# zchuning/repo

Measured on AMD Instinct MI355X. Metric: world-model+imagine updates/sec (B=50,L=50,64x64x3), higher is better.
Workload: dtype f32

## Files before the change

### include/repo_hip.h

```cpp
#ifndef REPO_HIP_H
#define REPO_HIP_H

#include <stddef.h>
#include <stdint.h>

#ifdef __cplusplus
extern "C" {
#endif

#ifndef __HIP_PLATFORM_AMD__
typedef struct ihipStream_t* hipStream_t;
#endif

#define REPO_ABI_VERSION 14

#define REPO_OK 0
#define REPO_E_BADARG (-1)
#define REPO_E_SHAPE (-2)
#define REPO_E_ALIGN (-3)
#define REPO_E_WS_TOO_SMALL (-4)
#define REPO_E_ARCH (-5)
#define REPO_E_ENV (-6)

#define REPO_EPI_NONE 0
// ... 277 lines not shown
int repo_vdb_head_bwd(int64_t N, int64_t Z, const float* z, int64_t ldz, const float* eps, uint64_t noise_seed,
                      uint64_t noise_offset, const float* lat, const float* fc_w, const float* dd, const float* beta,
                      float kl_coef, const float* extra, float* dz, int64_t lddz, float* dfc_w, float* dfc_b,
                      int accumulate, void* ws, size_t ws_bytes, hipStream_t stream);
int repo_vdb_beta_step(float* beta, const float* kl_real_sum, int64_t n_real, const float* kl_fake_sum, int64_t n_fake,
                       float beta_lr, float target_kl, float* kl_out, hipStream_t stream);
int repo_vdb_gp_delta(int64_t N, int64_t Z, const float* z, int64_t ldz, const float* eps, uint64_t noise_seed,
                      uint64_t noise_offset, const float* lat, const float* fc_w, float* delta5, int64_t lddelta,
                      hipStream_t stream);
int repo_vdb_gp_norm(int64_t n, float* g, float scale, float* sq_sum, void* ws, size_t ws_bytes, hipStream_t stream);
int repo_vdb_gp_head(int64_t N, int64_t Z, const float* a5, int64_t lda5, const float* z, int64_t ldz, const float* eps,
                     uint64_t noise_seed, uint64_t noise_offset, const float* lat, const float* fc_w, float* extra,
                     float* dfc_w, int accumulate, void* ws, size_t ws_bytes, hipStream_t stream);
int repo_vdb_tau(int64_t N, const float* lt, const float* d, const float* u, float* tau_out, float* dlt, float* sums,
                 void* ws, size_t ws_bytes, hipStream_t stream);

int repo_linear_unit_nll_fused(int64_t rows, int64_t O, int64_t K, const float* h, int64_t ldh, const float* W,
                               int64_t ldw);
int repo_linear_unit_nll(int64_t rows, int64_t O, int64_t K, const float* h, int64_t ldh, const float* W, int64_t ldw,
                         const float* bias, const float* target, int64_t ldt, float grad_scale, float* sums, float* dpre,
                         int64_t lddpre, float* recon, int64_t ldrecon, float* scratch, size_t scratch_bytes, void* ws,
                         size_t ws_bytes, hipStream_t stream);
int repo_debug_linear_nll(int mode);

int repo_film_fwd(int64_t nimg, int64_t C, int64_t P, const float* y, const float* film, int64_t ldfilm,
                  int64_t gamma_off, int64_t beta_off, float* out, hipStream_t stream);
int repo_film_bwd(int64_t nimg, int64_t C, int64_t P, const float* dh, const float* y, const float* film,
                  int64_t ldfilm, int64_t gamma_off, int64_t beta_off, float* dy, float* dfilm, hipStream_t stream);
int repo_film_tables(int64_t nimg, int nlayers, const int* channels, const float* film, int64_t ldfilm, float* tables,
                     hipStream_t stream);
int repo_film_bwd_h(int64_t nimg, int64_t C, int64_t P, const float* dh, const float* h, const float* film,
                    int64_t ldfilm, int64_t gamma_off, int64_t beta_off, float* dy, float* dfilm, int conv_kind,
                    const int64_t* geo, const void* x, int x_is_u8, const float* w, const float* bias,
                    unsigned* gated_epoch, unsigned epoch, hipStream_t stream);
size_t repo_kl_balance_tasks_workspace_bytes(void);
int repo_kl_balance_tasks(int64_t rows, int64_t S, int64_t C, const float* pm, const float* ps, const float* qm,
                          const float* qs, float alpha, const float* log_beta, const float* tasks, float target_kl,
                          float scale, float* dpm, float* dps, float* dqm, float* dqs, float* sums, void* ws,
                          size_t ws_bytes, hipStream_t stream);
int repo_dual_step_tasks(int64_t C, float* log_beta, float* exp_avg, float* exp_avg_sq, const float* sums,
                         int64_t rows, float lr, float beta1, float beta2, float eps, int64_t step, int apply,
                         float* scalars_out, const unsigned* skip_if_nonzero, hipStream_t stream);

int repo_transpose(int64_t rows, int64_t cols, const float* src, int64_t lds, float* dst, int64_t ldd,
                   hipStream_t stream);
int repo_gemm_nt_pays(int64_t M, int64_t N, int64_t K);

size_t repo_grad_sqnorm_workspace_bytes(void);
int repo_grad_sqnorm(int64_t n, const float* g, float* sqnorm, void* ws, size_t ws_bytes,
                     hipStream_t stream);
int repo_clip_adam(int64_t n, float* params, const float* grads, float* exp_avg, float* exp_avg_sq,
                   const float* sqnorm, float max_norm, float lr, float beta1, float beta2, float eps,
                   int64_t step, const unsigned* skip_if_nonzero, hipStream_t stream);

#ifdef __cplusplus
}
#endif
#endif
```

### repo_amd/algorithms/repo/dreamer.py

```python
import functools
import glob
import math
import os

import numpy as np
import torch

from ... import functional as Fn
from ... import ops
from ...common.buffers import SequenceReplayBuffer
from ...common.utils import get_device, postprocess, to_np
from .models.actor_critic import ActorModel, ValueModel
from .models.decoder import ContinuationModel, ObservationModel, RewardModel
from .models.encoder import Encoder
from .models.rssm import TransitionModel
from .models.utils import FlatAdam, InverseDynamicsModel
from .rollout import EpisodeDriver

LOG_2PI = math.log(2.0 * math.pi)


def _d(ts):
    return [t.detach() for t in ts]

# ... 279 lines not shown
        if self._pcont:
            self._pcont_backward(feat, st["pc_hid"], st["dpc"], dfeat)
        pd, gd = self._pg(self.obs_model)
        pr, gr = self._pg(self.transition_model)
        pe, ge = self._pg(self.encoder)
        dembeds = torch.empty(rows, self.c.embedding_size, device=dev)
        dpm, dps, dqm, dqs = kl_grads
        if self._symbolic:
            Fn.symbolic_decoder_bwd(pd, feat, st["dec_saved"], gd, self.obs_model.act,
                                    dfeat=dfeat if decoder_attached else None, accumulate_dfeat=True)
            self._model_bucket_begin(tail=True)
            ops.rssm_observe_bwd(pr, sv, gr, dfeat=dfeat, dpm=dpm, dps=dps, dqm=dqm, dqs=dqs, dembeds=dembeds,
                                 min_std=self.transition_model.min_std_dev)
            Fn.symbolic_encoder_bwd(pe, st["frames"], st["enc_saved"], dembeds, ge, self.encoder.act)
            return
        if decoder_attached:
            wgrads = []
            Fn.decoder_bwd(pd, feat, st["dec_saved"], gd, dfeat=dfeat, accumulate_dfeat=True, deferred=wgrads)
            main = torch.cuda.current_stream(dev)
            side = self._side_stream or main
            side.wait_stream(main)
            with torch.cuda.stream(side):
                ops.rssm_observe_bwd(pr, sv, gr, dfeat=dfeat, dpm=dpm, dps=dps, dqm=dqm, dqs=dqs, dembeds=dembeds,
                                     min_std=self.transition_model.min_std_dev)
            for fn in wgrads:
                fn()
            main.wait_stream(side)
            self._model_bucket_begin(tail=True)
            Fn.encoder_bwd(pe, st["frames"], st["enc_saved"], dembeds, ge, side=wside)
            return
        main = torch.cuda.current_stream(dev)
        side = self._side_stream or main
        side.wait_stream(main)
        with torch.cuda.stream(side):
            ops.rssm_observe_bwd(pr, sv, gr, dfeat=dfeat, dpm=dpm, dps=dps, dqm=dqm, dqs=dqs, dembeds=dembeds,
                                 min_std=self.transition_model.min_std_dev)
        Fn.decoder_bwd(pd, feat, st["dec_saved"], gd, side=wside)
        main.wait_stream(side)
        self._model_bucket_begin(tail=True)
        Fn.encoder_bwd(pe, st["frames"], st["enc_saved"], dembeds, ge, side=wside)

    def _model_bucket_begin(self, tail):
        if self.dp is None or not self._dp_two_buckets:
            return
        g, cut = self.model_optimizer.grad, self._model_cut
        if not tail:
            self._allreduce(g[:cut])
            return
        self._model_works.append(self.dp.all_reduce_begin(g[cut:], stream=self._side_stream))

    def _steppers(self):
        return [v for v in vars(self).values() if hasattr(v, "step_count") and hasattr(v, "exp_avg")]

    def _take_status(self):
        st = self._status_ring[self._update_seq % 8 : self._update_seq % 8 + 1]
        ops.take_status_into(ops.scan_status(self.device), st)
        if self.dp is not None:
            self.dp.all_reduce_status(st)
        self._ustatus = st
        for opt in self._steppers():
            opt.skip = st
        return st

    def _model_step(self):
        self._take_status()
        if self._ev_ac_done is not None:
            torch.cuda.current_stream(self.device).wait_event(self._ev_ac_done)
        if self.dp is not None and self._dp_two_buckets:
            self._model_bucket_begin(tail=False)
            works, self._model_works = self._model_works, []
            assert len(works) == 1, "model gradient buckets: the decoder bucket was not started by the backward"
            self.dp.all_reduce_end(works)
        elif self.dp is not None:
            self._allreduce(self.model_optimizer.grad)
        self.model_optimizer.clip_and_step(self.c.grad_clip_norm)

    def _prep_batch(self, obs, actions, rewards, nonterms):
        self._update_seq += 1
        self._restore_point = (self._update_seq, self._noise_counter, [(o, o.step_count) for o in self._steppers()])
        obs = obs.contiguous()
        assert obs.dtype in (torch.uint8, torch.float32), obs.dtype
        return obs, actions.float().contiguous(), rewards.float().contiguous(), nonterms.float().contiguous()

    @in_conv_precision
    def train_dynamics(self, obs, actions, rewards, nonterms):
        c = self.c
        obs, actions, rewards, nonterms = self._prep_batch(obs, actions, rewards, nonterms)
        st = self._world_model_forward(obs, actions, rewards, nonterms)
        sv, grow = st["sv"], st["grow"]
        if sv.prior_ready is not None:
            torch.cuda.current_stream(self.device).wait_stream(sv.prior_ready)
        kl_sum, kl_grads = ops.kl_balance(sv.prior_mean, sv.prior_std, sv.post_mean, sv.post_std, 1, 0.0, None,
                                          float(c.free_nats), 1.0 / grow)
        self._world_model_backward(st, kl_grads, decoder_attached=True)
        self._model_step()
        self._pending_model = (torch.cat([st["nll_sum"], st["rew_sums"], kl_sum, self.model_optimizer.sqnorm]), None,
                               grow)
        return self._latents_out(sv, actions, nonterms)

    def _latents_out(self, sv, actions, nonterms):
        D = self.c.belief_size
        beliefs, states = sv.featx[1:, :, :D], sv.featx[1:, :, D:]
        if self._inv_dyn:
            self.train_inv_dynamics(beliefs, states, actions, nonterms)
        return beliefs, states

    def train_inv_dynamics(self, beliefs, states, actions, nonterms):
        c = self.c
        m, opt = self.inv_dynamics, self.inv_dynamics_optimizer
        T, B, D = beliefs.shape
        S = states.shape[2]
        rows = beliefs.as_strided((T, B, D + S), beliefs.stride()) if (
            states.data_ptr() == beliefs.data_ptr() + 4 * D and states.stride() == beliefs.stride()
            and beliefs.stride(1) >= D + S) else torch.cat((beliefs, states), dim=2)
        x = ops.inv_dyn_pack(rows, D)
        N = x.shape[0]
        p, g = self._pg(m)
        raw, hid = ops.mlp_fwd(p, x, act=m.act)
        target, mask = actions[1:-1].reshape(N, -1), nonterms[1:-1].reshape(N)
        if self.dp is None:
            sums, draw = ops.normal_nll_rows(raw, target, mask, m.min_std_dev)
        else:
            sums, _ = ops.normal_nll_rows(raw, target, mask, m.min_std_dev, want_grad=False)
            total = sums.clone()
            self._allreduce(total)
            _, draw = ops.normal_nll_rows(raw, target, mask, m.min_std_dev, count_in=total[1:2])
        ops.mlp_bwd(p, x, hid, draw, dparams=g, dx=None, act=m.act)
        self._allreduce(opt.grad)
# ... 432 lines not shown
```

### repo_amd/algorithms/repo/models/utils.py

```python
import torch
import torch.nn as nn
import torch.nn.functional as F

from .... import ops


def bottle(f, xs):
    horizon, batch_size = xs[0].shape[:2]
    ys = f(*(x.reshape(horizon * batch_size, *x.shape[2:]) for x in xs))
    if isinstance(ys, tuple):
        return tuple(y.reshape(horizon, batch_size, *y.shape[1:]) for y in ys)
    return ys.reshape(horizon, batch_size, *ys.shape[1:])


class InverseDynamicsModel(nn.Module):

    def __init__(self, belief_size, state_size, action_size, hidden_size, activation_function="relu", min_std_dev=0.1):
        super().__init__()
        self.act = ops.dense_act_id(activation_function, type(self).__name__)
        self.min_std_dev = min_std_dev
        self.fc1 = nn.Linear(belief_size + state_size + belief_size, hidden_size)
        self.fc2 = nn.Linear(hidden_size, hidden_size)
        self.fc3 = nn.Linear(hidden_size, hidden_size)
        self.fc4 = nn.Linear(hidden_size, 2 * action_size)

    def plist(self):
        return [t for m in (self.fc1, self.fc2, self.fc3, self.fc4) for t in (m.weight, m.bias)]

    @torch.no_grad()
    def forward(self, belief, state, next_belief):
        x = torch.cat((belief, state, next_belief), dim=1).float().contiguous()
        raw, _ = ops.mlp_fwd([t.detach() for t in self.plist()], x, act=self.act)
        mean, std_dev = torch.chunk(raw, chunks=2, dim=1)
        return mean, F.softplus(std_dev) + self.min_std_dev


def adam_param_group(lr, betas, eps, n_params):
    probe = torch.optim.Adam([torch.nn.Parameter(torch.zeros(1))], lr=float(lr), betas=tuple(betas), eps=float(eps))
    group = dict(probe.state_dict()["param_groups"][0])
    group["params"] = list(range(n_params))
    return group


class FlatAdam:

    @staticmethod
    def padded_numel(params):
        return sum((p.numel() + 3) // 4 * 4 for p in params)

    def __init__(self, params, lr, betas=(0.9, 0.999), eps=1e-8, grad=None):
        self.params = list(params)
        assert self.params, "FlatAdam needs at least one parameter"
        self.lr, self.betas, self.eps = float(lr), tuple(betas), float(eps)
        self.step_count = 0
        dev = self.params[0].device
        sizes = [p.numel() for p in self.params]
        self.offsets, off = [], 0
        for n in sizes:
            self.offsets.append(off)
            off += (n + 3) // 4 * 4
        self.numel = off
        self.flat = torch.zeros(off, dtype=torch.float32, device=dev)
        if grad is None:
            grad = torch.zeros(off, dtype=torch.float32, device=dev)
        assert grad.shape == (off,) and grad.dtype == torch.float32 and grad.is_contiguous(), (grad.shape, off)
        self.grad = grad
        self.exp_avg = torch.zeros(off, dtype=torch.float32, device=dev)
        self.exp_avg_sq = torch.zeros(off, dtype=torch.float32, device=dev)
        self.sqnorm = torch.zeros(1, dtype=torch.float32, device=dev)
        self.skip = None
        self.gviews = []
        with torch.no_grad():
            for p, o, n in zip(self.params, self.offsets, sizes):
                self.flat[o : o + n].copy_(p.detach().reshape(-1))
                p.data = self.flat[o : o + n].view(p.shape)
                gv = self.grad[o : o + n].view(p.shape)
                p.grad = gv
                self.gviews.append(gv)

    @classmethod
    def view(cls, parent, n_params, lr):
        self = cls.__new__(cls)
        self.params = parent.params[:n_params]
        self.lr, self.betas, self.eps = float(lr), parent.betas, parent.eps
        self.step_count = 0
        self.offsets = parent.offsets[:n_params]
        self.numel = parent.offsets[n_params] if n_params < len(parent.params) else parent.numel
        self.flat, self.grad = parent.flat[: self.numel], parent.grad[: self.numel]
        self.exp_avg = torch.zeros_like(self.flat)
        self.exp_avg_sq = torch.zeros_like(self.flat)
        self.sqnorm = torch.zeros(1, dtype=torch.float32, device=self.flat.device)
        self.skip = None
        self.gviews = parent.gviews[:n_params]
        return self

    def zero_grad(self, set_to_none=False):
        self.grad.zero_()

    def clip_and_step(self, max_norm):
        self.step_count += 1
        ops.grad_sqnorm(self.grad, out=self.sqnorm)
        ops.clip_adam(self.flat, self.grad, self.exp_avg, self.exp_avg_sq, self.sqnorm, max_norm, self.lr,
                      self.step_count, self.betas, self.eps, skip=self.skip)

    def step(self):
        self.step_count += 1
        ops.clip_adam(self.flat, self.grad, self.exp_avg, self.exp_avg_sq, None, 0.0, self.lr, self.step_count,
                      self.betas, self.eps, skip=self.skip)

    def state_dict(self):
        state = {}
        if self.step_count > 0:
            for i, (p, o) in enumerate(zip(self.params, self.offsets)):
                n = p.numel()
                state[i] = {
                    "step": torch.tensor(float(self.step_count)),
                    "exp_avg": self.exp_avg[o : o + n].view(p.shape).clone(),
                    "exp_avg_sq": self.exp_avg_sq[o : o + n].view(p.shape).clone(),
                }
        return {"state": state, "param_groups": [adam_param_group(self.lr, self.betas, self.eps, len(self.params))]}

    def load_state_dict(self, sd):
        g = sd["param_groups"][0]
        self.lr, self.betas, self.eps = float(g["lr"]), tuple(g["betas"]), float(g["eps"])
        steps = set()
        with torch.no_grad():
            for i, (p, o) in enumerate(zip(self.params, self.offsets)):
                st = sd["state"].get(i)
                if st is None:
                    continue
                n = p.numel()
                self.exp_avg[o : o + n].copy_(st["exp_avg"].reshape(-1))
                self.exp_avg_sq[o : o + n].copy_(st["exp_avg_sq"].reshape(-1))
                steps.add(int(float(st["step"])))
        assert len(steps) <= 1, "per-parameter step counts differ; not an Adam state this optimiser can hold"
        self.step_count = steps.pop() if steps else 0
```

### repo_amd/algorithms/repo/repo.py

```python
import os

import numpy as np
import torch

from ... import functional as Fn
from ... import ops
from .dreamer import Dreamer, in_conv_precision
from .models.utils import adam_param_group


class _ScalarAdam:

    def __init__(self, param, lr, betas=(0.9, 0.999), eps=1e-8):
        self.param = param
        self.lr, self.betas, self.eps = float(lr), tuple(betas), float(eps)
        self.step_count = 0
        self.exp_avg = torch.zeros(1, dtype=torch.float32, device=param.device)
        self.exp_avg_sq = torch.zeros(1, dtype=torch.float32, device=param.device)

    def state_dict(self):
        state = {}
        if self.step_count > 0:
            state[0] = {"step": torch.tensor(float(self.step_count)), "exp_avg": self.exp_avg.reshape(()).clone(),
                        "exp_avg_sq": self.exp_avg_sq.reshape(()).clone()}
# ... 14 lines not shown
        super().build_models(config, env)
        self.log_beta = torch.tensor(np.log(config.init_beta), dtype=torch.float, device=self.device)
        self.beta_optimizer = _ScalarAdam(self.log_beta, lr=self.c.beta_lr)
        self._dual_out = torch.zeros(4, dtype=torch.float32, device=self.device)

    def _train_dynamics_split(self, obs, actions, rewards, nonterms):
        c, dev = self.c, self.device
        L, B = obs.shape[:2]
        T = L - 1
        rows = T * B
        grow = self._global_rows(rows)
        D, S = c.belief_size, c.state_size
        frames = obs[1:].reshape(rows, *obs.shape[2:])
        pe, ge = self._pg(self.encoder)
        embeds, enc_saved = Fn.encoder_fwd(pe, frames)
        pr, gr = self._pg(self.transition_model)
        pd, gd = self._pg(self.obs_model)
        head = Fn.dec_head_compose(pd) if Fn._dec_compose(rows, pd) else None
        sv = ops.rssm_observe_fwd(
            pr, *self._zero_state(B), actions[:-1].contiguous(),
            nonterms[:-1].reshape(T, B).contiguous(), embeds.view(T, B, -1), self._noise("obs_prior", (T, B, S)),
            self._noise("obs_post", (T, B, S)), self.transition_model.min_std_dev, noise=self._draw(2 * T * B * S),
            act=self.transition_model.act)
        feat = sv.featx[1:].reshape(rows, D + S)
        pw, gw = self._pg(self.reward_model)
        r_pred, r_hid = ops.mlp_fwd(pw, feat, act=self.reward_model.act)
        rew_sums, drew = ops.scalar_nll(r_pred.view(-1), rewards[:-1].reshape(-1).contiguous(),
                                        nonterms[:-1].reshape(-1).contiguous(), 1.0 / grow)
        if self._pcont:
            pc_hid, dpc = self._pcont_forward(feat, nonterms, grow)
        alpha = c.prior_train_steps / (1 + c.prior_train_steps)
        kl_sum, klg = ops.kl_balance(sv.prior_mean, sv.prior_std, sv.post_mean, sv.post_std, 0, alpha, self.log_beta, 0.0,
                                     1.0 / grow)
        main, side = torch.cuda.current_stream(dev), self._side_stream
        side.wait_stream(main)
        with torch.cuda.stream(side):
            dfeat = torch.empty(rows, D + S, device=dev)
            ops.mlp_bwd(pw, feat, r_hid, drew.view(rows, 1), dparams=gw, dx=dfeat, act=self.reward_model.act)
            if self._pcont:
                self._pcont_backward(feat, pc_hid, dpc, dfeat)
            ev_rew = torch.cuda.Event()
            ev_rew.record(side)
            dembeds = torch.empty(rows, c.embedding_size, device=dev)
            ops.rssm_observe_bwd(pr, sv, gr, dfeat=dfeat, dpm=klg[0], dps=klg[1], dqm=klg[2], dqs=klg[3], dembeds=dembeds,
                                 min_std=self.transition_model.min_std_dev)
            Fn.encoder_bwd(pe, frames, enc_saved, dembeds, ge, side=None)
        nll_sum, dec_saved = Fn.decoder_fwd_nll(pd, feat, frames, 1.0 / grow, head=head)
        Fn.decoder_bwd(pd, feat, dec_saved, gd, side=self._wgrad_side(B))
        if self.dp is not None and self._dp_two_buckets:
            main.wait_event(ev_rew)
            g, cut = self.model_optimizer.grad, self._model_cut
            self._model_works.append(self.dp.all_reduce_begin(g[cut:], stream=main))
        main.wait_stream(side)
        self._model_step()
        kl_global = kl_sum
        if self.dp is not None:
            kl_global = kl_sum.clone()
            self._allreduce(kl_global)
        bo = self.beta_optimizer
        bo.step_count += 1
        ops.dual_step(self.log_beta, bo.exp_avg, bo.exp_avg_sq, kl_global, grow, c.target_kl, bo.lr, bo.step_count,
                      betas=bo.betas, eps=bo.eps, out=self._dual_out, skip=self._ustatus)
        self._pending_model = (torch.cat([nll_sum, rew_sums, kl_sum, self.model_optimizer.sqnorm]), self._dual_out.clone(),
                               grow)
        return self._latents_out(sv, actions, nonterms)

    @in_conv_precision
    def train_dynamics(self, obs, actions, rewards, nonterms):
        c = self.c
        obs, actions, rewards, nonterms = self._prep_batch(obs, actions, rewards, nonterms)
        if os.environ.get("REPO_WM_SPLIT", "1") == "1" and self._side_stream is not None and not self._symbolic:
            return self._train_dynamics_split(obs, actions, rewards, nonterms)
        st = self._world_model_forward(obs, actions, rewards, nonterms)
        sv, grow = st["sv"], st["grow"]
        alpha = c.prior_train_steps / (1 + c.prior_train_steps)
        if sv.prior_ready is not None:
            torch.cuda.current_stream(self.device).wait_stream(sv.prior_ready)
        kl_sum, kl_grads = ops.kl_balance(sv.prior_mean, sv.prior_std, sv.post_mean, sv.post_std, 0, alpha,
                                          self.log_beta, 0.0, 1.0 / grow)
        self._world_model_backward(st, kl_grads, decoder_attached=False)
        self._model_step()
        kl_global = kl_sum
        if self.dp is not None:
            kl_global = kl_sum.clone()
            self._allreduce(kl_global)
        bo = self.beta_optimizer
        bo.step_count += 1
        ops.dual_step(self.log_beta, bo.exp_avg, bo.exp_avg_sq, kl_global, grow, c.target_kl, bo.lr, bo.step_count,
                      betas=bo.betas, eps=bo.eps, out=self._dual_out, skip=self._ustatus)
        self._pending_model = (torch.cat([st["nll_sum"], st["rew_sums"], kl_sum, self.model_optimizer.sqnorm]),
                               self._dual_out.clone(), grow)
        return self._latents_out(sv, actions, nonterms)

    def get_param_dict(self):
        params = super().get_param_dict()
        params["log_beta"] = self.log_beta.detach().clone().requires_grad_(True)
        params["beta_optimizer"] = self.beta_optimizer.state_dict()
        return params

    def load_param_dict(self, params):
        super().load_param_dict(params)
        with torch.no_grad():
            self.log_beta.copy_(params["log_beta"].to(self.device))
        self.beta_optimizer.load_state_dict(params["beta_optimizer"])
```

### repo_amd/csrc/common.h

```cpp
#pragma once
#include <hip/hip_runtime.h>
#include <stdint.h>

#include "../../include/repo_hip.h"

#define REPO_CHECK_LAUNCH()                      \
  do {                                           \
    hipError_t _e = hipGetLastError();           \
    if (_e != hipSuccess) return (int)_e;        \
  } while (0)

#define REPO_ARCH_GUARD()                 \
  do {                                    \
    int _a = repo::arch_status();         \
    if (_a != REPO_OK) return _a;         \
  } while (0)

#define REPO_REQUIRE(cond, code) \
  do {                           \
    if (!(cond)) return (code);  \
  } while (0)

namespace repo {

// ... 26 lines not shown
__device__ __forceinline__ float pix_norm(uint8_t v) { return ((float)v / 255.f) * 2.f - 1.f; }

__device__ __forceinline__ float load_as_float(const float* p, unsigned i) { return p[i]; }
__device__ __forceinline__ float load_as_float(const uint8_t* p, unsigned i) { return pix_norm(p[i]); }

__device__ __forceinline__ float wave_sum(float v) {
#pragma unroll
  for (int o = 32; o > 0; o >>= 1) v += __shfl_xor(v, o, 64);
  return v;
}
__device__ __forceinline__ double wave_sum_d(double v) {
#pragma unroll
  for (int o = 32; o > 0; o >>= 1) v += __shfl_xor(v, o, 64);
  return v;
}

__device__ __forceinline__ float block_sum(float v, float* smem ) {
  v = wave_sum(v);
  const int lane = threadIdx.x & 63, wid = threadIdx.x >> 6;
  if (lane == 0) smem[wid] = v;
  __syncthreads();
  float r = 0.f;
  if (threadIdx.x == 0) {
    const int nw = (blockDim.x + 63) >> 6;
    for (int i = 0; i < nw; ++i) r += smem[i];
  }
  __syncthreads();
  return r;
}

constexpr int kRedHeaderBytes = 256;
constexpr int kLastBlockMaxGrid = 64;
__device__ __forceinline__ void last_block_finishes(const float* parts, int nvals, float* out, unsigned* ticket, float* smem) {
  if (!ticket) return;
  __shared__ int s_last;
  __threadfence();
  __syncthreads();
  if (threadIdx.x == 0)
    s_last = __hip_atomic_fetch_add(ticket, 1u, __ATOMIC_RELAXED, __HIP_MEMORY_SCOPE_AGENT) == gridDim.x - 1;
  __syncthreads();
  if (!s_last) return;
  __threadfence();
  const int n = gridDim.x;
  for (int v = 0; v < nvals; ++v) {
    float s = 0.f;
    for (int i = threadIdx.x; i < n; i += blockDim.x)
      s += __hip_atomic_load(parts + v * n + i, __ATOMIC_RELAXED, __HIP_MEMORY_SCOPE_AGENT);
    s = block_sum(s, smem);
    if (threadIdx.x == 0) out[v] = s;
  }
  if (threadIdx.x == 0) __hip_atomic_store(ticket, 0u, __ATOMIC_RELAXED, __HIP_MEMORY_SCOPE_AGENT);
}

inline int cdiv(long a, long b) { return (int)((a + b - 1) / b); }

__device__ __forceinline__ void philox4x32_10(unsigned (&c)[4], unsigned k0, unsigned k1) {
#pragma unroll
  for (int r = 0; r < 10; ++r) {
    const unsigned h0 = __umulhi(0xD2511F53u, c[0]), l0 = 0xD2511F53u * c[0];
    const unsigned h1 = __umulhi(0xCD9E8D57u, c[2]), l1 = 0xCD9E8D57u * c[2];
    const unsigned n0 = h1 ^ c[1] ^ k0, n2 = h0 ^ c[3] ^ k1;
    c[0] = n0; c[1] = l1; c[2] = n2; c[3] = l0;
    k0 += 0x9E3779B9u; k1 += 0xBB67AE85u;
  }
}
__device__ __forceinline__ void philox_normal4(uint64_t seed, uint64_t blk, float (&z)[4]) {
  unsigned c[4] = {(unsigned)blk, (unsigned)(blk >> 32), 0u, 0u};
  philox4x32_10(c, (unsigned)seed, (unsigned)(seed >> 32));
#pragma unroll
  for (int h = 0; h < 2; ++h) {
    const float u1 = ((float)(c[2 * h] >> 8) + 0.5f) * (1.f / 16777216.f);
    const float u2 = ((float)(c[2 * h + 1] >> 8) + 0.5f) * (1.f / 16777216.f);
    const float rad = __builtin_amdgcn_sqrtf(-1.3862943611198906f * __builtin_amdgcn_logf(u1));
    z[2 * h] = rad * __builtin_amdgcn_cosf(u2);
    z[2 * h + 1] = rad * __builtin_amdgcn_sinf(u2);
  }
}
__device__ __forceinline__ float philox_normal(uint64_t seed, uint64_t i) {
  float z[4];
  philox_normal4(seed, i >> 2, z);
  const int l = (int)(i & 3);
  return l == 0 ? z[0] : l == 1 ? z[1] : l == 2 ? z[2] : z[3];
}
struct NoiseSrc {
  const float* p;
  uint64_t seed, base;
  __device__ __forceinline__ float at(size_t i) const { return p ? p[i] : philox_normal(seed, base + i); }
};

constexpr int kMaxWgradGroup = 9;
struct WgradDesc {
  int64_t M, N, K;
  const float* dY;
  int64_t lddy;
  const float* X;
  int64_t ldx;
  float* dW;
  int64_t lddw;
  float* db;
};
size_t gemm_wgrad_group_ws_bytes(const WgradDesc* d, int n);
int gemm_wgrad_group(const WgradDesc* d, int n, int accumulate, void* ws, size_t ws_bytes, hipStream_t stream);

}
```

### repo_amd/csrc/loss.hip

```cpp
#include "common.h"

namespace repo {

constexpr int kRedBlocks = 1024;

__global__ void final_sum_kernel(const float* __restrict__ parts, int n, int nvals, float* __restrict__ out) {
  __shared__ float red[16];
  for (int v = 0; v < nvals; ++v) {
    float s = 0.f;
    for (int i = threadIdx.x; i < n; i += blockDim.x) s += parts[v * n + i];
    s = block_sum(s, red);
    if (threadIdx.x == 0) out[v] = s;
  }
}

__global__ __launch_bounds__(256) void kl_kernel(int rows, int S, const float* __restrict__ pm,
                                                 const float* __restrict__ ps, const float* __restrict__ qm,
                                                 const float* __restrict__ qs, int mode, float alpha,
                                                 const float* __restrict__ log_beta, float free_nats, float scale,
                                                 float* __restrict__ dpm, float* __restrict__ dps,
                                                 float* __restrict__ dqm, float* __restrict__ dqs,
                                                 float* __restrict__ parts, float* __restrict__ red_out,
    unsigned* __restrict__ ticket) {
  __shared__ float red[16];
  const int lane = threadIdx.x & 63, wid = threadIdx.x >> 6, nw = blockDim.x >> 6;
  const float beta = (mode == 0 && log_beta) ? expf(*log_beta) : 1.f;
  float acc = 0.f;
  for (int row = blockIdx.x * nw + wid; row < rows; row += gridDim.x * nw) {
    float kl = 0.f, gpm = 0.f, gps = 0.f, gqm = 0.f, gqs = 0.f;
    const size_t o = (size_t)row * S + lane;
    if (lane < S) {
      const float mp = pm[o], sp = ps[o], mq = qm[o], sq = qs[o];
      const float ratio = sq / sp, vr = ratio * ratio;
      const float dm = (mq - mp) / sp, t1 = dm * dm;
      kl = 0.5f * (vr + t1 - 1.f - logf(vr));
      const float isp2 = 1.f / (sp * sp);
      gqm = (mq - mp) * isp2;
      gpm = -gqm;
      gqs = -1.f / sq + sq * isp2;
      gps = 1.f / sp - (sq * sq + (mq - mp) * (mq - mp)) * isp2 / sp;
    }
    const float klrow = wave_sum(kl);
    float wp, wq;
    if (mode == 0) {
      wp = beta * alpha * scale;
      wq = beta * (1.f - alpha) * scale;
      if (lane == 0) acc += klrow;
    } else {
      const bool active = klrow > free_nats;
      wp = wq = active ? scale : klrow == free_nats ? 0.5f * scale : 0.f;
      if (lane == 0) acc += active ? klrow : free_nats;
    }
    if (lane < S) {
      if (dpm) dpm[o] = gpm * wp;
      if (dps) dps[o] = gps * wp;
      if (dqm) dqm[o] = gqm * wq;
      if (dqs) dqs[o] = gqs * wq;
    }
  }
  const float s = block_sum(acc, red);
  if (threadIdx.x == 0) parts[blockIdx.x] = s;
  last_block_finishes(parts, 1, red_out, ticket, red);
}

__global__ void dual_step_kernel(float* __restrict__ log_beta, float* __restrict__ m, float* __restrict__ v,
                                 const float* __restrict__ kl_sum, float inv_rows, float target_kl, float lr, float b1,
                                 float b2, float eps, float bc1, float bc2_sqrt, int apply,
                                 float* __restrict__ scalars_out, const unsigned* __restrict__ skip) {
  if (threadIdx.x != 0 || blockIdx.x != 0) return;
  if (skip && *skip) apply = 0;
  const float lb = *log_beta;
  const float kl_div = *kl_sum * inv_rows;
  const float viol = kl_div - target_kl;
  const float g = -viol;
  scalars_out[0] = kl_div;
  scalars_out[1] = expf(lb) * viol;
  scalars_out[2] = -lb * viol;
  float nlb = lb;
  if (apply) {
    const float mm = b1 * (*m) + (1.f - b1) * g;
    const float vv = b2 * (*v) + (1.f - b2) * g * g;
    *m = mm;
    *v = vv;
    nlb = lb - (lr / bc1) * mm / (sqrtf(vv) / bc2_sqrt + eps);
    *log_beta = nlb;
  }
  scalars_out[3] = expf(nlb);
}

__global__ __launch_bounds__(256) void scalar_nll_kernel(int n, const float* __restrict__ pred,
                                                         const float* __restrict__ target,
                                                         const float* __restrict__ mask, float scale,
                                                         float* __restrict__ dpred, float* __restrict__ parts, float* __restrict__ red_out,
    unsigned* __restrict__ ticket) {
  __shared__ float red[16];
  float a = 0.f, msum = 0.f;
  for (int i = blockIdx.x * blockDim.x + threadIdx.x; i < n; i += gridDim.x * blockDim.x) {
    const float mk = mask ? mask[i] : 1.f;
    const float d = pred[i] - target[i];
    a += 0.5f * d * d * mk;
    msum += mk;
    if (dpred) dpred[i] = d * mk * scale;
  }
  const float s0 = block_sum(a, red);
  const float s1 = block_sum(msum, red);
  if (threadIdx.x == 0) {
    parts[blockIdx.x] = s0;
    parts[gridDim.x + blockIdx.x] = s1;
  }
  last_block_finishes(parts, 2, red_out, ticket, red);
}

__global__ __launch_bounds__(256) void tanh_normal_entropy_kernel(int n, int NS, const float* __restrict__ mean,
                                                                  const float* __restrict__ stdv,
                                                                  const float* __restrict__ eps, uint64_t nseed,
                                                                  uint64_t noffset, float gscale,
                                                                  float* __restrict__ dmean, float* __restrict__ dstd,
                                                                  float* __restrict__ parts, float* __restrict__ red_out,
    unsigned* __restrict__ ticket) {
  __shared__ float red[16];
  const float kClamp = 0.99999994f;
  const float kLog2 = 0.69314718055994531f;
  float acc = 0.f;
  for (int e = blockIdx.x * blockDim.x + threadIdx.x; e < n; e += gridDim.x * blockDim.x) {
    const float mu = mean[e], sd = stdv[e];
    const float isd = 1.f / sd, isd2 = isd * isd, lsd = __logf(sd);
    float slog = 0.f, gmu = 0.f, gsd = 0.f;
    float z[4];
    const uint64_t first = noffset + (uint64_t)e * NS;
    for (int s = 0; s < NS; ++s) {
      float ep;
      if (eps) {
        ep = eps[(size_t)s * n + e];
      } else {
        const uint64_t i = first + s;
        if (s == 0 || (i & 3) == 0) philox_normal4(nseed, i >> 2, z);
        const int l = (int)(i & 3);
        ep = l == 0 ? z[0] : l == 1 ? z[1] : l == 2 ? z[2] : z[3];
      }
      const float u = fmaf(sd, ep, mu);
// ... 463 lines not shown
```

### repo_amd/csrc/optim.hip

```cpp
#include "common.h"

namespace repo {

__global__ __launch_bounds__(256) void sqnorm_kernel(int64_t n, const float* __restrict__ g, float* __restrict__ parts) {
  __shared__ float red[16];
  float acc = 0.f;
  const int64_t stride = (int64_t)gridDim.x * blockDim.x * 4;
  for (int64_t i = ((int64_t)blockIdx.x * blockDim.x + threadIdx.x) * 4; i < n; i += stride) {
    if (i + 3 < n) {
      const float4 v = *reinterpret_cast<const float4*>(g + i);
      acc += v.x * v.x + v.y * v.y + v.z * v.z + v.w * v.w;
    } else {
      for (int64_t j = i; j < n; ++j) acc += g[j] * g[j];
    }
  }
  const float s = block_sum(acc, red);
  if (threadIdx.x == 0) parts[blockIdx.x] = s;
}

__global__ void sqnorm_final_kernel(const float* __restrict__ parts, int n, float* __restrict__ out) {
  __shared__ float red[16];
  float s = 0.f;
  for (int i = threadIdx.x; i < n; i += blockDim.x) s += parts[i];
  s = block_sum(s, red);
  if (threadIdx.x == 0) *out = s;
}

__global__ __launch_bounds__(256) void clip_adam_kernel(int64_t n, float* __restrict__ p, const float* __restrict__ g,
                                                        float* __restrict__ m, float* __restrict__ v,
                                                        const float* __restrict__ sqnorm, float max_norm, float lr_bc1,
                                                        float b1, float b2, float eps, float inv_bc2_sqrt,
                                                        const unsigned* __restrict__ skip) {
  if (skip && *skip) return;
  float coef = 1.f;
  if (sqnorm) {
    coef = max_norm / (sqrtf(*sqnorm) + 1e-6f);
    coef = coef > 1.f ? 1.f : coef;
  }
  const int64_t stride = (int64_t)gridDim.x * blockDim.x;
  for (int64_t i = (int64_t)blockIdx.x * blockDim.x + threadIdx.x; i < n; i += stride) {
    const float gg = g[i] * coef;
    const float mm = b1 * m[i] + (1.f - b1) * gg;
    const float vv = b2 * v[i] + (1.f - b2) * gg * gg;
    m[i] = mm;
    v[i] = vv;
    p[i] = p[i] - lr_bc1 * (mm / (sqrtf(vv) * inv_bc2_sqrt + eps));
  }
}

}

using namespace repo;

extern "C" size_t repo_grad_sqnorm_workspace_bytes(void) { return kRedHeaderBytes + 1024 * sizeof(float); }

extern "C" int repo_grad_sqnorm(int64_t n, const float* g, float* sqnorm, void* ws, size_t ws_bytes,
                                hipStream_t stream) {
  REPO_ARCH_GUARD();
  REPO_REQUIRE(n > 0, REPO_E_SHAPE);
  REPO_REQUIRE(g && sqnorm, REPO_E_BADARG);
  REPO_REQUIRE(((uintptr_t)g & 15) == 0, REPO_E_ALIGN);
  REPO_REQUIRE(ws && ws_bytes >= repo_grad_sqnorm_workspace_bytes(), REPO_E_WS_TOO_SMALL);
  long blocks = (n + 4095) / 4096;
  if (blocks > 1024) blocks = 1024;
  float* parts = (float*)((char*)ws + kRedHeaderBytes);
  hipLaunchKernelGGL(sqnorm_kernel, dim3((unsigned)blocks), dim3(256), 0, stream, n, g, parts);
  REPO_CHECK_LAUNCH();
  hipLaunchKernelGGL(sqnorm_final_kernel, dim3(1), dim3(256), 0, stream, (const float*)parts, (int)blocks, sqnorm);
  REPO_CHECK_LAUNCH();
  return REPO_OK;
}

extern "C" int repo_clip_adam(int64_t n, float* params, const float* grads, float* exp_avg, float* exp_avg_sq,
                              const float* sqnorm, float max_norm, float lr, float beta1, float beta2, float eps,
                              int64_t step, const unsigned* skip_if_nonzero, hipStream_t stream) {
  REPO_ARCH_GUARD();
  REPO_REQUIRE(n > 0 && step >= 1, REPO_E_SHAPE);
  REPO_REQUIRE(params && grads && exp_avg && exp_avg_sq, REPO_E_BADARG);
  const double bc1 = 1.0 - pow((double)beta1, (double)step);
  const double bc2 = 1.0 - pow((double)beta2, (double)step);
  long blocks = (n + 255) / 256;
  if (blocks > 2048) blocks = 2048;
  hipLaunchKernelGGL(clip_adam_kernel, dim3((unsigned)blocks), dim3(256), 0, stream, n, params, grads, exp_avg,
                     exp_avg_sq, sqnorm, max_norm, (float)((double)lr / bc1), beta1, beta2, eps,
                     (float)(1.0 / sqrt(bc2)), skip_if_nonzero);
  REPO_CHECK_LAUNCH();
  return REPO_OK;
}
```

### repo_amd/ops.py

```python
import contextlib
import os
import threading

import torch

from ._lib import check, lib

EPI_NONE, EPI_ELU, EPI_RELU, EPI_MUL_DELU, EPI_MUL_DRELU, EPI_MUL_MASK4, EPI_MUL_CMASK, EPI_FILM_RELU = 0, 1, 2, 3, 4, 5, 6, 7
EPI_LEAKY, EPI_MUL_DLEAKY = 8, 9
ACT_ELU, ACT_RELU = 0, 1
DENSE_ACTIVATIONS = {"elu": ACT_ELU, "relu": ACT_RELU}


def dense_act_id(name, what):
    try:
        return DENSE_ACTIVATIONS[name]
    except (KeyError, TypeError):
        raise NotImplementedError(
            f"{what}: the HIP dense kernels are built for dense_activation_function 'elu' or 'relu', not {name!r}") from None


def _saved_act(sv, act):
    if act is not None and act != sv.act:
        raise ValueError(f"backward asked for activation {act}, the forward ran with {sv.act}")
# ... 892 lines not shown
def bernoulli_nll(logit, base, target_scale, scale, want_grad=True, out=None):
    n = logit.numel()
    dev = logit.device
    assert base.numel() == n
    dlogit = torch.empty(n, dtype=torch.float32, device=dev) if want_grad else None
    if out is None:
        out = torch.empty(1, dtype=torch.float32, device=dev)
    ws = reduce_ws(dev)
    check(
        lib().repo_bernoulli_nll(n, _ptr(_f32c(logit)), _ptr(_f32c(base)), float(target_scale), float(scale),
                                 _ptr(dlogit), _ptr(out), _ptr(ws), ws.numel(), _stream()),
        "repo_bernoulli_nll",
    )
    return out, dlogit


def lambda_return_disc(rewards, values, disc, lambda_, gret=0.0, disc_is_logit=False, want_grads=True):
    Hm, N = rewards.shape
    dev = rewards.device
    assert values.shape == (Hm, N) and disc.shape == (Hm, N)
    returns = torch.empty(max(Hm - 1, 0), N, dtype=torch.float32, device=dev)
    weights = torch.empty(max(Hm - 1, 0), N, dtype=torch.float32, device=dev)
    dr, dv, dd = ([torch.empty(Hm, N, dtype=torch.float32, device=dev) for _ in range(3)] if want_grads
                  else [None] * 3)
    out = torch.empty(2, dtype=torch.float32, device=dev)
    ws = reduce_ws(dev)
    check(
        lib().repo_lambda_return_disc(Hm, N, _ptr(_f32c(rewards)), _ptr(_f32c(values)), _ptr(_f32c(disc)),
                                      int(bool(disc_is_logit)), float(lambda_), float(gret), _ptr(returns),
                                      _ptr(weights), _ptr(dr), _ptr(dv), _ptr(dd), _ptr(out), _ptr(ws), ws.numel(),
                                      _stream()),
        "repo_lambda_return_disc",
    )
    return returns, weights, dr, dv, dd, out


def grad_sqnorm(g, out=None):
    if out is None:
        out = torch.empty(1, dtype=torch.float32, device=g.device)
    ws = reduce_ws(g.device, lib().repo_grad_sqnorm_workspace_bytes())
    check(lib().repo_grad_sqnorm(g.numel(), _ptr(_f32c(g)), _ptr(out), _ptr(ws), ws.numel(), _stream()),
          "repo_grad_sqnorm")
    return out


def clip_adam(p, g, m, v, sqnorm, max_norm, lr, step, betas=(0.9, 0.999), eps=1e-8, skip=None):
    check(
        lib().repo_clip_adam(p.numel(), _ptr(_f32c(p)), _ptr(_f32c(g)), _ptr(_f32c(m)), _ptr(_f32c(v)), _ptr(sqnorm),
                             float(max_norm), float(lr), betas[0], betas[1], eps, step, _ptr(skip), _stream()),
        "repo_clip_adam",
    )


def philox_normal(n, seed, offset, device):
    out = torch.empty(int(n), dtype=torch.float32, device=device)
    check(lib().repo_philox_normal(_ptr(out), int(n), int(seed), int(offset), _stream()), "repo_philox_normal")
    return out


def film_fwd(y, film, gamma_off, beta_off, out=None):
    n, C = y.shape[:2]
    P = y.numel() // (n * C)
    if out is None:
        out = torch.empty_like(y)
    check(lib().repo_film_fwd(n, C, P, _ptr(y), _ptr(film), film.shape[1], gamma_off, beta_off, _ptr(out), _stream()),
          "repo_film_fwd")
    return out


def film_tables(film, channels):
    n = film.shape[0]
    assert film.shape[1] >= 2 * sum(channels) and film.is_contiguous() and 1 <= len(channels) <= 4
    buf = torch.empty(n * 2 * sum(channels), dtype=torch.float32, device=film.device)
    arr = (ctypes.c_int * len(channels))(*channels)
    check(lib().repo_film_tables(n, len(channels), arr, _ptr(film), film.shape[1], _ptr(buf), _stream()), "repo_film_tables")
    out, o = [], 0
    for c in channels:
        out.append(buf[o : o + n * 2 * c].view(n, 2, c))
        o += n * 2 * c
    return out


FILM_CONV_DOWN, FILM_CONV_UP, FILM_DENSE = 1, 2, 3


def film_bwd_h(dh, h, film, gamma_off, beta_off, dfilm, dy=None, exact=None, epoch_word=True):
    n, C = h.shape[:2]
    P = h.numel() // (n * C)
    if dy is None:
        dy = torch.empty_like(h)
    kind, geo, x, w, bias = 0, None, None, None, None
    if exact is not None:
        kind, which, x, w, bias = exact
        dense = which if isinstance(which, tuple) else (which, False)
        if kind == FILM_DENSE:
            geo4 = (int(dense[0]), int(bool(dense[1])), 0, 0)
        else:
            geo4 = tuple(int(v) for v in which) if isinstance(which, tuple) else CONV_GEO[which]
        geo = (ctypes.c_int64 * 4)(*geo4)
        assert x.is_contiguous() and w.is_contiguous() and x.dtype in (torch.float32, torch.uint8)
    global _film_epoch
    _film_epoch = _film_epoch % 0xFFFFFFF0 + 1
    word = reduce_ws(h.device)[32:36] if epoch_word else None
    check(lib().repo_film_bwd_h(n, C, P, _ptr(dh), _ptr(h), _ptr(film), film.shape[1], gamma_off, beta_off, _ptr(dy),
                                _ptr(dfilm), kind, geo, _ptr(x), int(x is not None and x.dtype == torch.uint8),
                                _ptr(_f32c(w)) if w is not None else None, _ptr(bias), _ptr(word), _film_epoch,
# ... 144 lines not shown
```

Measured before the change: 178.2.

## Fuse model optimizer tail: status take, sqnorm final, clip-Adam, dual step, log packing

```diff
diff --git a/include/repo_hip.h b/include/repo_hip.h
--- a/include/repo_hip.h
+++ b/include/repo_hip.h
@@ -353,6 +353,15 @@
 int repo_clip_adam(int64_t n, float* params, const float* grads, float* exp_avg, float* exp_avg_sq,
                    const float* sqnorm, float max_norm, float lr, float beta1, float beta2, float eps,
                    int64_t step, const unsigned* skip_if_nonzero, hipStream_t stream);
+int repo_grad_sqnorm_take(int64_t n, const float* g, unsigned* sticky, unsigned* taken, void* ws, size_t ws_bytes,
+                          hipStream_t stream);
+int repo_model_tail(int64_t n, float* params, const float* grads, float* exp_avg, float* exp_avg_sq,
+                    const void* ws, size_t ws_bytes, float* sqnorm, float max_norm, float lr, float beta1,
+                    float beta2, float eps, int64_t step, const unsigned* skip_if_nonzero, float* log_beta,
+                    float* dual_exp_avg, float* dual_exp_avg_sq, const float* kl_dual, const float* kl_log,
+                    int64_t rows, float target_kl, float dual_lr, float dual_beta1, float dual_beta2,
+                    float dual_eps, int64_t dual_step, const float* nll_sum, const float* rew_sums2,
+                    float* log_out9, hipStream_t stream);
 
 #ifdef __cplusplus
 }
diff --git a/repo_amd/algorithms/repo/dreamer.py b/repo_amd/algorithms/repo/dreamer.py
--- a/repo_amd/algorithms/repo/dreamer.py
+++ b/repo_amd/algorithms/repo/dreamer.py
@@ -355,10 +355,12 @@
     def _steppers(self):
         return [v for v in vars(self).values() if hasattr(v, "step_count") and hasattr(v, "exp_avg")]
 
-    def _take_status(self):
+    def _take_status(self, in_step=False):
         st = self._status_ring[self._update_seq % 8 : self._update_seq % 8 + 1]
-        ops.take_status_into(ops.scan_status(self.device), st)
+        if not in_step:
+            ops.take_status_into(ops.scan_status(self.device), st)
         if self.dp is not None:
+            assert not in_step
             self.dp.all_reduce_status(st)
         self._ustatus = st
         for opt in self._steppers():
@@ -366,7 +368,11 @@
         return st
 
     def _model_step(self):
-        self._take_status()
+        self._model_step_sync()
+        self.model_optimizer.clip_and_step(self.c.grad_clip_norm)
+
+    def _model_step_sync(self, status_in_step=False):
+        self._take_status(in_step=status_in_step)
         if self._ev_ac_done is not None:
             torch.cuda.current_stream(self.device).wait_event(self._ev_ac_done)
         if self.dp is not None and self._dp_two_buckets:
@@ -376,7 +382,6 @@
             self.dp.all_reduce_end(works)
         elif self.dp is not None:
             self._allreduce(self.model_optimizer.grad)
-        self.model_optimizer.clip_and_step(self.c.grad_clip_norm)
 
     def _prep_batch(self, obs, actions, rewards, nonterms):
         self._update_seq += 1
diff --git a/repo_amd/algorithms/repo/models/utils.py b/repo_amd/algorithms/repo/models/utils.py
--- a/repo_amd/algorithms/repo/models/utils.py
+++ b/repo_amd/algorithms/repo/models/utils.py
@@ -69,6 +69,7 @@
         self.exp_avg_sq = torch.zeros(off, dtype=torch.float32, device=dev)
         self.sqnorm = torch.zeros(1, dtype=torch.float32, device=dev)
         self.skip = None
+        self.tail = self.tail_out = None
         self.gviews = []
         with torch.no_grad():
             for p, o, n in zip(self.params, self.offsets, sizes):
@@ -91,6 +92,7 @@
         self.exp_avg_sq = torch.zeros_like(self.flat)
         self.sqnorm = torch.zeros(1, dtype=torch.float32, device=self.flat.device)
         self.skip = None
+        self.tail = self.tail_out = None
         self.gviews = parent.gviews[:n_params]
         return self
 
@@ -99,9 +101,21 @@
 
     def clip_and_step(self, max_norm):
         self.step_count += 1
+        tail, self.tail = self.tail, None
+        if tail is not None:
+            self.tail_out = self._step_with_tail(max_norm, *tail)
+            return
         ops.grad_sqnorm(self.grad, out=self.sqnorm)
         ops.clip_adam(self.flat, self.grad, self.exp_avg, self.exp_avg_sq, self.sqnorm, max_norm, self.lr,
                       self.step_count, self.betas, self.eps, skip=self.skip)
+
+    def _step_with_tail(self, max_norm, dual, kl_dual, kl_log, rows, target_kl, nll_sum, rew_sums, status):
+        sticky, taken = status if status is not None else (None, None)
+        ops.grad_sqnorm_take(self.grad, sticky, taken)
+        return ops.model_tail(self.flat, self.grad, self.exp_avg, self.exp_avg_sq, self.sqnorm, max_norm, self.lr,
+                              self.step_count, self.betas, self.eps, self.skip, dual.param, dual.exp_avg,
+                              dual.exp_avg_sq, kl_dual, kl_log, rows, target_kl, dual.lr, dual.step_count, dual.betas,
+                              dual.eps, nll_sum, rew_sums)
 
     def step(self):
         self.step_count += 1
diff --git a/repo_amd/algorithms/repo/repo.py b/repo_amd/algorithms/repo/repo.py
--- a/repo_amd/algorithms/repo/repo.py
+++ b/repo_amd/algorithms/repo/repo.py
@@ -90,17 +90,27 @@
             g, cut = self.model_optimizer.grad, self._model_cut
             self._model_works.append(self.dp.all_reduce_begin(g[cut:], stream=main))
         main.wait_stream(side)
-        self._model_step()
+        bo, opt = self.beta_optimizer, self.model_optimizer
+        bo.step_count += 1
+        tail = os.environ.get("REPO_WM_TAIL", "1") == "1"
+        if tail:
+            self._model_step_sync(status_in_step=self.dp is None)
+        else:
+            self._model_step()
         kl_global = kl_sum
         if self.dp is not None:
             kl_global = kl_sum.clone()
             self._allreduce(kl_global)
-        bo = self.beta_optimizer
-        bo.step_count += 1
-        ops.dual_step(self.log_beta, bo.exp_avg, bo.exp_avg_sq, kl_global, grow, c.target_kl, bo.lr, bo.step_count,
-                      betas=bo.betas, eps=bo.eps, out=self._dual_out, skip=self._ustatus)
-        self._pending_model = (torch.cat([nll_sum, rew_sums, kl_sum, self.model_optimizer.sqnorm]), self._dual_out.clone(),
-                               grow)
+        if tail:
+            opt.tail = (bo, kl_global, kl_sum, grow, c.target_kl, nll_sum, rew_sums,
+                        (ops.scan_status(dev), self._ustatus) if self.dp is None else None)
+            opt.clip_and_step(c.grad_clip_norm)
+            out, opt.tail_out = opt.tail_out, None
+            self._pending_model = (out[:5], out[5:], grow)
+        else:
+            ops.dual_step(self.log_beta, bo.exp_avg, bo.exp_avg_sq, kl_global, grow, c.target_kl, bo.lr, bo.step_count,
+                          betas=bo.betas, eps=bo.eps, out=self._dual_out, skip=self._ustatus)
+            self._pending_model = (torch.cat([nll_sum, rew_sums, kl_sum, opt.sqnorm]), self._dual_out.clone(), grow)
         return self._latents_out(sv, actions, nonterms)
 
     @in_conv_precision
diff --git a/repo_amd/csrc/common.h b/repo_amd/csrc/common.h
--- a/repo_amd/csrc/common.h
+++ b/repo_amd/csrc/common.h
@@ -102,6 +102,29 @@
   if (threadIdx.x == 0) __hip_atomic_store(ticket, 0u, __ATOMIC_RELAXED, __HIP_MEMORY_SCOPE_AGENT);
 }
 
+__device__ __forceinline__ void dual_step_one(float* __restrict__ log_beta, float* __restrict__ m, float* __restrict__ v,
+                                              float kl_sum, float inv_rows, float target_kl, float lr, float b1, float b2,
+                                              float eps, float bc1, float bc2_sqrt, int apply,
+                                              float* __restrict__ scalars_out) {
+  const float lb = *log_beta;
+  const float kl_div = kl_sum * inv_rows;
+  const float viol = kl_div - target_kl;
+  const float g = -viol;
+  scalars_out[0] = kl_div;
+  scalars_out[1] = expf(lb) * viol;
+  scalars_out[2] = -lb * viol;
+  float nlb = lb;
+  if (apply) {
+    const float mm = b1 * (*m) + (1.f - b1) * g;
+    const float vv = b2 * (*v) + (1.f - b2) * g * g;
+    *m = mm;
+    *v = vv;
+    nlb = lb - (lr / bc1) * mm / (sqrtf(vv) / bc2_sqrt + eps);
+    *log_beta = nlb;
+  }
+  scalars_out[3] = expf(nlb);
+}
+
 inline int cdiv(long a, long b) { return (int)((a + b - 1) / b); }
 
 __device__ __forceinline__ void philox4x32_10(unsigned (&c)[4], unsigned k0, unsigned k1) {
diff --git a/repo_amd/csrc/loss.hip b/repo_amd/csrc/loss.hip
--- a/repo_amd/csrc/loss.hip
+++ b/repo_amd/csrc/loss.hip
@@ -69,23 +69,7 @@
                                  float* __restrict__ scalars_out, const unsigned* __restrict__ skip) {
   if (threadIdx.x != 0 || blockIdx.x != 0) return;
   if (skip && *skip) apply = 0;
-  const float lb = *log_beta;
-  const float kl_div = *kl_sum * inv_rows;
-  const float viol = kl_div - target_kl;
-  const float g = -viol;
-  scalars_out[0] = kl_div;
-  scalars_out[1] = expf(lb) * viol;
-  scalars_out[2] = -lb * viol;
-  float nlb = lb;
-  if (apply) {
-    const float mm = b1 * (*m) + (1.f - b1) * g;
-    const float vv = b2 * (*v) + (1.f - b2) * g * g;
-    *m = mm;
-    *v = vv;
-    nlb = lb - (lr / bc1) * mm / (sqrtf(vv) / bc2_sqrt + eps);
-    *log_beta = nlb;
-  }
-  scalars_out[3] = expf(nlb);
+  dual_step_one(log_beta, m, v, *kl_sum, inv_rows, target_kl, lr, b1, b2, eps, bc1, bc2_sqrt, apply, scalars_out);
 }
 
 __global__ __launch_bounds__(256) void scalar_nll_kernel(int n, const float* __restrict__ pred,
diff --git a/repo_amd/csrc/optim.hip b/repo_amd/csrc/optim.hip
--- a/repo_amd/csrc/optim.hip
+++ b/repo_amd/csrc/optim.hip
@@ -2,8 +2,13 @@
 
 namespace repo {
 
-__global__ __launch_bounds__(256) void sqnorm_kernel(int64_t n, const float* __restrict__ g, float* __restrict__ parts) {
+__global__ __launch_bounds__(256) void sqnorm_kernel(int64_t n, const float* __restrict__ g, float* __restrict__ parts,
+                                                     unsigned* __restrict__ sticky, unsigned* __restrict__ taken) {
   __shared__ float red[16];
+  if (sticky && blockIdx.x == 0 && threadIdx.x == 0) {
+    *taken = *sticky;
+    *sticky = 0u;
+  }
   float acc = 0.f;
   const int64_t stride = (int64_t)gridDim.x * blockDim.x * 4;
   for (int64_t i = ((int64_t)blockIdx.x * blockDim.x + threadIdx.x) * 4; i < n; i += stride) {
@@ -18,23 +23,25 @@
   if (threadIdx.x == 0) parts[blockIdx.x] = s;
 }
 
+__device__ __forceinline__ float sqnorm_final(const float* __restrict__ parts, int n, float* red) {
+  float s = 0.f;
+  for (int i = threadIdx.x; i < n; i += blockDim.x) s += parts[i];
+  return block_sum(s, red);
+}
+
 __global__ void sqnorm_final_kernel(const float* __restrict__ parts, int n, float* __restrict__ out) {
   __shared__ float red[16];
-  float s = 0.f;
-  for (int i = threadIdx.x; i < n; i += blockDim.x) s += parts[i];
-  s = block_sum(s, red);
+  const float s = sqnorm_final(parts, n, red);
   if (threadIdx.x == 0) *out = s;
 }
 
-__global__ __launch_bounds__(256) void clip_adam_kernel(int64_t n, float* __restrict__ p, const float* __restrict__ g,
-                                                        float* __restrict__ m, float* __restrict__ v,
-                                                        const float* __restrict__ sqnorm, float max_norm, float lr_bc1,
-                                                        float b1, float b2, float eps, float inv_bc2_sqrt,
-                                                        const unsigned* __restrict__ skip) {
-  if (skip && *skip) return;
+__device__ __forceinline__ void clip_adam_body(int64_t n, float* __restrict__ p, const float* __restrict__ g,
+                                               float* __restrict__ m, float* __restrict__ v,
+                                               bool clip, float sqnorm, float max_norm, float lr_bc1, float b1,
+                                               float b2, float eps, float inv_bc2_sqrt) {
   float coef = 1.f;
-  if (sqnorm) {
-    coef = max_norm / (sqrtf(*sqnorm) + 1e-6f);
+  if (clip) {
+    coef = max_norm / (sqrtf(sqnorm) + 1e-6f);
     coef = coef > 1.f ? 1.f : coef;
   }
   const int64_t stride = (int64_t)gridDim.x * blockDim.x;
@@ -48,9 +55,58 @@
   }
 }
 
+__global__ __launch_bounds__(256) void clip_adam_kernel(int64_t n, float* __restrict__ p, const float* __restrict__ g,
+                                                        float* __restrict__ m, float* __restrict__ v,
+                                                        const float* __restrict__ sqnorm, float max_norm, float lr_bc1,
+                                                        float b1, float b2, float eps, float inv_bc2_sqrt,
+                                                        const unsigned* __restrict__ skip) {
+  if (skip && *skip) return;
+  clip_adam_body(n, p, g, m, v, sqnorm != nullptr, sqnorm ? *sqnorm : 0.f, max_norm, lr_bc1, b1, b2, eps, inv_bc2_sqrt);
+}
+
+struct ModelTail {
+  float *log_beta, *dm, *dv;
+  const float *kl_dual, *kl_log;
+  const float *nll_sum, *rew_sums;
+  float* log_out;
+  float inv_rows, target_kl, lr, b1, b2, eps, bc1, bc2_sqrt;
+};
+
+__global__ __launch_bounds__(256) void model_tail_kernel(int64_t n, float* __restrict__ p, const float* __restrict__ g,
+                                                         float* __restrict__ m, float* __restrict__ v,
+                                                         const float* __restrict__ parts, int nparts,
+                                                         float* __restrict__ sqnorm_out, float max_norm, float lr_bc1,
+                                                         float b1, float b2, float eps, float inv_bc2_sqrt,
+                                                         const unsigned* __restrict__ skip, ModelTail t) {
+  __shared__ float red[16];
+  __shared__ float s_sq;
+  const float s = sqnorm_final(parts, nparts, red);
+  if (threadIdx.x == 0) s_sq = s;
+  __syncthreads();
+  const float sq = s_sq;
+  const bool skipped = skip && *skip;
+  if (blockIdx.x == 0 && threadIdx.x == 0) {
+    *sqnorm_out = sq;
+    t.log_out[0] = *t.nll_sum;
+    t.log_out[1] = t.rew_sums[0];
+    t.log_out[2] = t.rew_sums[1];
+    t.log_out[3] = *t.kl_log;
+    t.log_out[4] = sq;
+    dual_step_one(t.log_beta, t.dm, t.dv, *t.kl_dual, t.inv_rows, t.target_kl, t.lr, t.b1, t.b2, t.eps, t.bc1, t.bc2_sqrt,
+                  skipped ? 0 : 1, t.log_out + 5);
+  }
+  if (skipped) return;
+  clip_adam_body(n, p, g, m, v, true, sq, max_norm, lr_bc1, b1, b2, eps, inv_bc2_sqrt);
+}
+
 }
 
 using namespace repo;
+
+static inline long sqnorm_blocks(int64_t n) {
+  const long blocks = (long)((n + 4095) / 4096);
+  return blocks > 1024 ? 1024 : blocks;
+}
 
 extern "C" size_t repo_grad_sqnorm_workspace_bytes(void) { return kRedHeaderBytes + 1024 * sizeof(float); }
 
@@ -61,10 +117,10 @@
   REPO_REQUIRE(g && sqnorm, REPO_E_BADARG);
   REPO_REQUIRE(((uintptr_t)g & 15) == 0, REPO_E_ALIGN);
   REPO_REQUIRE(ws && ws_bytes >= repo_grad_sqnorm_workspace_bytes(), REPO_E_WS_TOO_SMALL);
-  long blocks = (n + 4095) / 4096;
-  if (blocks > 1024) blocks = 1024;
+  const long blocks = sqnorm_blocks(n);
   float* parts = (float*)((char*)ws + kRedHeaderBytes);
-  hipLaunchKernelGGL(sqnorm_kernel, dim3((unsigned)blocks), dim3(256), 0, stream, n, g, parts);
+  hipLaunchKernelGGL(sqnorm_kernel, dim3((unsigned)blocks), dim3(256), 0, stream, n, g, parts, (unsigned*)nullptr,
+                     (unsigned*)nullptr);
   REPO_CHECK_LAUNCH();
   hipLaunchKernelGGL(sqnorm_final_kernel, dim3(1), dim3(256), 0, stream, (const float*)parts, (int)blocks, sqnorm);
   REPO_CHECK_LAUNCH();
@@ -87,3 +143,47 @@
   REPO_CHECK_LAUNCH();
   return REPO_OK;
 }
+
+extern "C" int repo_grad_sqnorm_take(int64_t n, const float* g, unsigned* sticky, unsigned* taken, void* ws,
+                                     size_t ws_bytes, hipStream_t stream) {
+  REPO_ARCH_GUARD();
+  REPO_REQUIRE(n > 0, REPO_E_SHAPE);
+  REPO_REQUIRE(g && (!sticky == !taken) && (!sticky || sticky != taken), REPO_E_BADARG);
+  REPO_REQUIRE(((uintptr_t)g & 15) == 0, REPO_E_ALIGN);
+  REPO_REQUIRE(ws && ws_bytes >= repo_grad_sqnorm_workspace_bytes(), REPO_E_WS_TOO_SMALL);
+  hipLaunchKernelGGL(sqnorm_kernel, dim3((unsigned)sqnorm_blocks(n)), dim3(256), 0, stream, n, g,
+                     (float*)((char*)ws + kRedHeaderBytes), sticky, taken);
+  REPO_CHECK_LAUNCH();
+  return REPO_OK;
+}
+
+extern "C" int repo_model_tail(int64_t n, float* params, const float* grads, float* exp_avg, float* exp_avg_sq,
+                               const void* ws, size_t ws_bytes, float* sqnorm, float max_norm, float lr, float beta1,
+                               float beta2, float eps, int64_t step, const unsigned* skip_if_nonzero, float* log_beta,
+                               float* dual_exp_avg, float* dual_exp_avg_sq, const float* kl_dual, const float* kl_log,
+                               int64_t rows, float target_kl, float dual_lr, float dual_beta1, float dual_beta2,
+                               float dual_eps, int64_t dual_step, const float* nll_sum, const float* rew_sums2,
+                               float* log_out9, hipStream_t stream) {
+  REPO_ARCH_GUARD();
+  REPO_REQUIRE(n > 0 && step >= 1 && dual_step >= 1 && rows > 0, REPO_E_SHAPE);
+  REPO_REQUIRE(params && grads && exp_avg && exp_avg_sq && sqnorm, REPO_E_BADARG);
+  REPO_REQUIRE(log_beta && dual_exp_avg && dual_exp_avg_sq && kl_dual && kl_log && nll_sum && rew_sums2 && log_out9,
+               REPO_E_BADARG);
+  REPO_REQUIRE(ws && ws_bytes >= repo_grad_sqnorm_workspace_bytes(), REPO_E_WS_TOO_SMALL);
+  const double bc1 = 1.0 - pow((double)beta1, (double)step);
+  const double bc2 = 1.0 - pow((double)beta2, (double)step);
+  const double dbc1 = 1.0 - pow((double)dual_beta1, (double)dual_step);
+  const double dbc2 = 1.0 - pow((double)dual_beta2, (double)dual_step);
+  ModelTail t;
+  t.log_beta = log_beta; t.dm = dual_exp_avg; t.dv = dual_exp_avg_sq;
+  t.kl_dual = kl_dual; t.kl_log = kl_log; t.nll_sum = nll_sum; t.rew_sums = rew_sums2; t.log_out = log_out9;
+  t.inv_rows = (float)(1.0 / (double)rows); t.target_kl = target_kl; t.lr = dual_lr; t.b1 = dual_beta1; t.b2 = dual_beta2;
+  t.eps = dual_eps; t.bc1 = (float)dbc1; t.bc2_sqrt = (float)sqrt(dbc2);
+  long blocks = (n + 255) / 256;
+  if (blocks > 2048) blocks = 2048;
+  hipLaunchKernelGGL(model_tail_kernel, dim3((unsigned)blocks), dim3(256), 0, stream, n, params, grads, exp_avg,
+                     exp_avg_sq, (const float*)((const char*)ws + kRedHeaderBytes), (int)sqnorm_blocks(n), sqnorm,
+                     max_norm, (float)((double)lr / bc1), beta1, beta2, eps, (float)(1.0 / sqrt(bc2)), skip_if_nonzero, t);
+  REPO_CHECK_LAUNCH();
+  return REPO_OK;
+}
diff --git a/repo_amd/ops.py b/repo_amd/ops.py
--- a/repo_amd/ops.py
+++ b/repo_amd/ops.py
@@ -968,6 +968,28 @@
     )
 
 
+def grad_sqnorm_take(g, sticky=None, taken=None):
+    ws = reduce_ws(g.device, lib().repo_grad_sqnorm_workspace_bytes())
+    check(lib().repo_grad_sqnorm_take(g.numel(), _ptr(_f32c(g)), _ptr(sticky), _ptr(taken), _ptr(ws), ws.numel(),
+                                      _stream()), "repo_grad_sqnorm_take")
+
+
+def model_tail(p, g, m, v, sqnorm, max_norm, lr, step, betas, eps, skip, log_beta, dual_m, dual_v, kl_dual, kl_log, rows,
+               target_kl, dual_lr, dual_step_count, dual_betas, dual_eps, nll_sum, rew_sums, out=None):
+    if out is None:
+        out = torch.empty(9, dtype=torch.float32, device=p.device)
+    ws = reduce_ws(g.device, lib().repo_grad_sqnorm_workspace_bytes())
+    check(
+        lib().repo_model_tail(p.numel(), _ptr(_f32c(p)), _ptr(_f32c(g)), _ptr(_f32c(m)), _ptr(_f32c(v)), _ptr(ws),
+                              ws.numel(), _ptr(sqnorm), float(max_norm), float(lr), betas[0], betas[1], eps, step,
+                              _ptr(skip), _ptr(log_beta), _ptr(dual_m), _ptr(dual_v), _ptr(kl_dual), _ptr(kl_log), rows,
+                              float(target_kl), float(dual_lr), dual_betas[0], dual_betas[1], dual_eps, dual_step_count,
+                              _ptr(nll_sum), _ptr(rew_sums), _ptr(out), _stream()),
+        "repo_model_tail",
+    )
+    return out
+
+
 def philox_normal(n, seed, offset, device):
     out = torch.empty(int(n), dtype=torch.float32, device=device)
     check(lib().repo_philox_normal(_ptr(out), int(n), int(seed), int(offset), _stream()), "repo_philox_normal")
```

Result: no change. 178.6, median of 6 (+0.3%).
